# scenarios/VAE-2

Hardware: AMD Instinct MI355X
Metric: training frames/sec on 128x256 8-frame Cityscapes clips, 1/2/4/8 MI355X (higher is better)
Workload: dtype fp32; 1 GPU; VAE2 ELBO step (encz + encoder + 2 decoders fwd/bwd + Adam), HRNet-W18-small-v2, 128x256, 8 clips/GPU x 9 frames (CLIP_LENGTH=3); yaml=vae-2_amd/experiments/vae2_w18_small_v2_128x256.yaml, global_batch=8, frames_per_clip=9, parallelism=dp1, sync_bn=False, launch=hip_graph, mfma_operands=fp32

## Files before the change

### include/vae2_hip.h

```cpp
#ifndef VAE2_HIP_H
#define VAE2_HIP_H

#include <stdint.h>

#ifdef __cplusplus
extern "C" {
#endif

typedef struct vae2_act {
  int64_t n, h, w, c;
  int64_t ps;
} vae2_act;

#define VAE2_ABI_VERSION 15

int vae2_abi_version(void);
const char* vae2_last_error(void);

int vae2_kernel_log(int enable);
int64_t vae2_kernel_log_read(char* buf, int64_t len);


int64_t vae2_conv2d_fwd_stats_rows(const float* x, const vae2_act* xd, const vae2_act* yd,
                                   int k, int stride, int pad);
// ... 157 lines not shown
} vae2_bn_layer;
int vae2_bn_multi_apply(int n, const vae2_bn_layer* layers, void* stream);
int vae2_bn_multi_bwd_reduce(int n, const vae2_bn_layer* layers, void* stream);
int vae2_bn_multi_bwd_apply(int n, const vae2_bn_layer* layers, void* stream);

typedef struct vae2_bn_fin {
  const float* partials; int64_t rows; int64_t c;
  double* sums;
  const double* countp;
  double count;
  const float* gamma; const float* beta;
  float* running_mean; float* running_var; int64_t* num_batches_tracked;
  float momentum, eps;
  float* save;
  float* dgamma; float* dbeta;
} vae2_bn_fin;
int vae2_bn_multi_reduce(int n, const vae2_bn_fin* fins, int mode, void* stream);
int vae2_bn_multi_finalize(int n, const vae2_bn_fin* fins, void* stream);

int64_t vae2_conv1x1_upsum_stats_rows(const vae2_act* yd);
int vae2_conv1x1_upsum_fwd(const float* x, const vae2_act* xd, const float* wp,
                           const float* bias, int nup, const float* const* ups,
                           const vae2_act* upds, float* y, const vae2_act* yd, float* stats,
                           void* stream);

int vae2_head_out_fwd(const float* y, const vae2_act* yd, const float* save, const float* w2,
                      const float* b2, int cout2, float* out, const vae2_act* outd,
                      void* stream);
int64_t vae2_head_out_bwd_ws_size(const vae2_act* yd, int cout2);
int vae2_head_out_bwd_reduce(const float* y, const vae2_act* yd, const float* save,
                             const float* w2, int cout2, const float* dout,
                             const vae2_act* doutd, double* sums, float* dgamma, float* dbeta,
                             float* dw2, float* db2, float* ws, int64_t ws_size, void* stream);
int vae2_head_out_bwd_apply(const float* y, const vae2_act* yd, const float* save,
                            const float* gamma, const float* w2, int cout2, const float* dout,
                            const vae2_act* doutd, const double* sums, double count, float* dy,
                            const vae2_act* dyd, float* dbias, float* ws, int64_t ws_size,
                            void* stream);


int vae2_upsample_bilinear_fwd(const float* x, const vae2_act* xd, float* y,
                               const vae2_act* yd, float beta, void* stream);
int vae2_upsample_bilinear_bwd(const float* dy, const vae2_act* dyd, float* dx,
                               const vae2_act* dxd, float beta, void* stream);

int vae2_fuse_sum_relu(int n, const float* const* xs, const vae2_act* xds,
                       float* y, const vae2_act* yd, void* stream);
int vae2_fuse_sum_relu_bn(int n, const float* const* xs, const vae2_act* xds,
                          const float* const* saves, float* y, const vae2_act* yd,
                          void* stream);

int vae2_heads_set_algo(int algo);

int64_t vae2_upsample_bilinear_bwd_multi_ws_size(const vae2_act* dyd, int n,
                                                 const vae2_act* dxds);
int vae2_upsample_bilinear_bwd_multi(const float* dy, const vae2_act* dyd, int n,
                                     float* const* dxs, const vae2_act* dxds, float* ws,
                                     int64_t ws_size, void* stream);

int64_t vae2_upsample_bilinear_bwd_pow2_ws_size(const vae2_act* dyd, int n,
                                                const vae2_act* dxds);
int vae2_upsample_bilinear_bwd_pow2(const float* dy, const vae2_act* dyd, int n,
                                    float* const* dxs, const vae2_act* dxds,
                                    const float* betas, float* ws, int64_t ws_size,
                                    void* stream);

int vae2_relu_bwd(const float* dy, const vae2_act* dyd, const float* y,
                  const vae2_act* yd, float* g, const vae2_act* gd,
                  void* stream);

int vae2_relu_bwd_dual(const float* dy, const vae2_act* dyd, const float* y,
                       const vae2_act* yd, float* g, const vae2_act* gd, float* g2,
                       const vae2_act* g2d, float beta2, void* stream);

int vae2_copy_act(const float* x, const vae2_act* xd, float* y,
                  const vae2_act* yd, float beta, void* stream);

int vae2_codemap_tile_fwd(const float* v, int64_t vs, float* y,
                          const vae2_act* yd, void* stream);
int64_t vae2_spatial_ws_size(const vae2_act* xd);
int vae2_codemap_tile_bwd(const float* dy, const vae2_act* dyd, float* dv,
                          int64_t vs, int accumulate, float* ws, int64_t ws_size,
                          void* stream);

int vae2_nchw_to_nhwc(const float* x, float* y, const vae2_act* yd,
                      float beta, void* stream);
int vae2_nhwc_to_nchw(const float* x, const vae2_act* xd, float* y,
                      float beta, void* stream);

int vae2_global_avgpool_fwd(const float* x, const vae2_act* xd, float* y,
                            const vae2_act* yd, float* ws, int64_t ws_size,
                            void* stream);
int vae2_global_avgpool_bwd(const float* dy, const vae2_act* dyd, float* dx,
                            const vae2_act* dxd, float beta, void* stream);
int vae2_weighted_avgpool_fwd(const float* x, const vae2_act* xd, const float* wr,
                              const float* wc, float scale, float* y, const vae2_act* yd,
                              float* ws, int64_t ws_size, void* stream);
int vae2_weighted_avgpool_bwd(const float* dy, const vae2_act* dyd, const float* wr,
                              const float* wc, float scale, float* dx, const vae2_act* dxd,
                              float beta, void* stream);


int64_t vae2_reduce_ws_size(int64_t n);
int vae2_l1_fwd(const float* p, const vae2_act* pd, const float* t,
                const vae2_act* td, float scale, float* ws, float* out,
                void* stream);
// ... 107 lines not shown
```

### vae-2_amd/csrc/heads.hip

```cpp
#include "common.h"

namespace vae2 {


constexpr int kHeadMaxOut = 4;
constexpr int64_t kHeadMaxPpb = 2048;

template <int CO>
__device__ __forceinline__ void head_stage_dout(float* sd, const float* dout, const Act& dod,
                                                int64_t p0, int64_t p1) {
  const int n = (int)(p1 - p0) * CO;
  for (int i = threadIdx.x; i < n; i += 256) {
    const int pp = i / CO, o = i - pp * CO;
    sd[i] = dout[(p0 + pp) * dod.ps + o];
  }
}

__device__ __forceinline__ f4 hld4(const float* p) { return *reinterpret_cast<const f4*>(p); }

__device__ __forceinline__ const float* yb_at(const float* y, int64_t P, int64_t p, int c) {
  return y + (int64_t)(c >> 6) * P * 64 + p * 64 + (c & 63);
}

__device__ __forceinline__ f4 hchan4(const float* a, int c, int C) {
// ... 1072 lines not shown
int adj3_fuse_launch(const float* dy, const vae2_act* dyd, int n, float* const* dxs,
                     const vae2_act* dxds, const float* betas, hipStream_t st) {
  if (!g_adj_fused || !g_fuse_adj3 || n < 1 || n > 3 || !adj_one_pass(dyd, n, dxds)) return -1;
  for (int s = 0; s < n; ++s)
    if (!dxs[s] || dxds[s].n != dyd->n || dxds[s].c != dyd->c) return -1;
  UpAdj p{};
  p.dy = dy; p.dy_ps = (int)dyd->ps; p.H = (int)dyd->h; p.W = (int)dyd->w; p.C = (int)dyd->c;
  for (int s = 0; s < n; ++s) {
    p.dx[s] = dxs[s]; p.zh[s] = (int)dxds[s].h; p.zw[s] = (int)dxds[s].w;
    p.dx_ps[s] = (int)dxds[s].ps;
    p.beta[s] = betas ? betas[s] : 0.f;
  }
  p.nxb = (int)ceil_div(dyd->w, kUsXB);
  const int br = dyd->h < g_adj_band ? (int)dyd->h : g_adj_band;
  const int nband = (int)ceil_div(dyd->h, br);
  const dim3 grid((unsigned)(dyd->n * nband * p.nxb * ceil_div(dyd->c, 64)));
  switch (n) {
    case 1: VAE2_LAUNCH(up_adj3_kernel<1>, grid, dim3(256), 0, st, p, br, nband); break;
    case 2: VAE2_LAUNCH(up_adj3_kernel<2>, grid, dim3(256), 0, st, p, br, nband); break;
    default: VAE2_LAUNCH(up_adj3_kernel<3>, grid, dim3(256), 0, st, p, br, nband); break;
  }
  return 0;
}

static int64_t head_ppb(int64_t P, int64_t blocks = 2048) {
  int64_t ppb = ceil_div(P, blocks);
  ppb = ppb < 64 ? 64 : ppb;
  return ppb > kHeadMaxPpb ? kHeadMaxPpb : ppb;
}

static bool head_args_ok(const float* y, const vae2_act* yd, int cout2) {
  return y && act_ok(yd) && ((uintptr_t)y % 16 == 0) && (yd->c + 3) / 4 <= 256 &&
         cout2 >= 1 && cout2 <= kHeadMaxOut;
}

#define HEAD_DISPATCH(CO_, KERNEL, ...)                                   \
  switch (CO_) {                                                          \
    case 1: VAE2_LAUNCH((KERNEL<1>), __VA_ARGS__); break;          \
    case 2: VAE2_LAUNCH((KERNEL<2>), __VA_ARGS__); break;          \
    case 3: VAE2_LAUNCH((KERNEL<3>), __VA_ARGS__); break;          \
    default: VAE2_LAUNCH((KERNEL<4>), __VA_ARGS__); break;         \
  }
#define HEAD_DISPATCH_U(CO_, U_, KERNEL, ...)                                  \
  if ((U_) == 4) {                                                             \
    switch (CO_) {                                                             \
      case 1: VAE2_LAUNCH((KERNEL<1, 4>), __VA_ARGS__); break;                 \
      case 2: VAE2_LAUNCH((KERNEL<2, 4>), __VA_ARGS__); break;                 \
      case 3: VAE2_LAUNCH((KERNEL<3, 4>), __VA_ARGS__); break;                 \
      default: VAE2_LAUNCH((KERNEL<4, 4>), __VA_ARGS__); break;                \
    }                                                                          \
  } else {                                                                     \
    HEAD_DISPATCH(CO_, KERNEL, __VA_ARGS__)                                    \
  }

}

using namespace vae2;

extern "C" {

int vae2_head_out_fwd(const float* y, const vae2_act* yd, const float* save, const float* w2,
                      const float* b2, int cout2, float* out, const vae2_act* outd,
                      void* stream) {
  const char* fn = "vae2_head_out_fwd";
  VAE2_REQUIRE(head_args_ok(y, yd, cout2) && save && w2 && out && act_ok(outd), fn,
               "bad arguments (y must be 16-byte aligned NHWC with ps % 4 == 0, cout2 <= 4)");
  VAE2_REQUIRE(outd->n == yd->n && outd->h == yd->h && outd->w == yd->w && outd->c >= cout2,
               fn, "output shape mismatch");
  const int c4 = (int)((yd->c + 3) / 4);
  const size_t shm = (size_t)(2 + cout2) * c4 * 16;
  const int64_t P = act_pixels(yd);
  const unsigned grid = (unsigned)(ceil_div(P, 16) < 8192 ? ceil_div(P, 16) : 8192);
  HEAD_DISPATCH(cout2, head_out_fwd_kernel, dim3(grid), dim3(256), shm, as_stream(stream), y,
                to_act(yd), save, w2, b2, out, to_act(outd));
  return check_launch(fn);
}

int64_t vae2_head_out_bwd_ws_size(const vae2_act* yd, int cout2) {
  if (!act_ok(yd)) return 0;
  const int64_t P = act_pixels(yd);
  const int64_t blocks = ceil_div(P, head_ppb(P));
  const int64_t NC = 2 * yd->c + cout2 * yd->c + cout2;
  return blocks * NC;
}

int vae2_head_out_bwd_reduce(const float* y, const vae2_act* yd, const float* save,
                             const float* w2, int cout2, const float* dout,
                             const vae2_act* doutd, double* sums, float* dgamma, float* dbeta,
                             float* dw2, float* db2, float* ws, int64_t ws_size, void* stream) {
  const char* fn = "vae2_head_out_bwd_reduce";
  VAE2_REQUIRE(head_args_ok(y, yd, cout2) && save && w2 && dout && sums && ws &&
                   act_ok(doutd), fn, "bad arguments");
  VAE2_REQUIRE(doutd->n == yd->n && doutd->h == yd->h && doutd->w == yd->w &&
                   doutd->c >= cout2, fn, "dout shape mismatch");
  VAE2_REQUIRE(ws_size >= vae2_head_out_bwd_ws_size(yd, cout2), fn, "workspace too small");
  const int C = (int)yd->c, c4 = (C + 3) / 4, rows = 256 / c4;
  const int NC = 2 * C + cout2 * C + cout2;
  const int64_t P = act_pixels(yd), ppb = head_ppb(P);
  const unsigned blocks = (unsigned)ceil_div(P, ppb);
  const size_t shm = ((size_t)rows * NC + (size_t)ppb * cout2) * sizeof(float);
  VAE2_REQUIRE(shm <= 64 * 1024, fn, "too many channels for the LDS reduction");
  HEAD_DISPATCH_U(cout2, g_head_red_u, head_out_bwd_reduce_kernel, dim3(blocks), dim3(256), shm,
                as_stream(stream), y, to_act(yd), save, w2, dout, to_act(doutd), ppb, rows, ws);
  int rc = check_launch(fn);
  if (rc) return rc;
  VAE2_LAUNCH(head_bwd_colsum_kernel, dim3((unsigned)ceil_div(NC, 64)), dim3(1024), 0,
// ... 79 lines not shown
  dim3 grid((unsigned)(yd->n * p.nrb * p.nxb * ncb));
  hipStream_t st = as_stream(stream);
  bool one = g_upsum_one && yd->w % kUsXB == 0 && p.cin4 <= 20;
  for (int s = 0; s < nup; ++s)
    one = one && yd->h == (int64_t)p.zh[s] << (s + 1) && yd->w == (int64_t)p.zw[s] << (s + 1);
  if (one) {
#define US2_LAUNCH(N)                                                                   \
  switch (p.cin4 / 4) {                                                                 \
    case 1: VAE2_LAUNCH((upsum2_kernel<N, 1>), grid, dim3(256), 0, st, p); break;       \
    case 2: VAE2_LAUNCH((upsum2_kernel<N, 2>), grid, dim3(256), 0, st, p); break;       \
    case 3: VAE2_LAUNCH((upsum2_kernel<N, 3>), grid, dim3(256), 0, st, p); break;       \
    case 4: VAE2_LAUNCH((upsum2_kernel<N, 4>), grid, dim3(256), 0, st, p); break;       \
    default: VAE2_LAUNCH((upsum2_kernel<N, 5>), grid, dim3(256), 0, st, p); break;      \
  }
    switch (nup) {
      case 0: US2_LAUNCH(0) break;
      case 1: US2_LAUNCH(1) break;
      case 2: US2_LAUNCH(2) break;
      default: US2_LAUNCH(3) break;
    }
#undef US2_LAUNCH
    return check_launch(fn);
  }
  bool tight = g_upsum_tight != 0;
  for (int s = 0; s < nup; ++s) tight = tight && p.vcols[s] <= 4 * us_vu(s, true);
  const bool kq5 = p.cin4 <= 20;
#define US_LAUNCH(N)                                                                    \
  if (tight && kq5) VAE2_LAUNCH((upsum_kernel<N, true, 5>), grid, dim3(256), shm, st, p); \
  else if (tight) VAE2_LAUNCH((upsum_kernel<N, true, 8>), grid, dim3(256), shm, st, p); \
  else VAE2_LAUNCH((upsum_kernel<N, false, 8>), grid, dim3(256), shm, st, p);
  switch (nup) {
    case 0: US_LAUNCH(0) break;
    case 1: US_LAUNCH(1) break;
    case 2: US_LAUNCH(2) break;
    default: US_LAUNCH(3) break;
  }
#undef US_LAUNCH
  return check_launch(fn);
}

int64_t vae2_upsample_bilinear_bwd_multi_ws_size(const vae2_act* dyd, int n,
                                                 const vae2_act* dxds) {
  if (!act_ok(dyd) || n < 0 || n > 3 || (n && !dxds)) return 0;
  if (adj_one_pass(dyd, n, dxds)) return 1;
  int64_t t = 0;
  for (int s = 0; s < n; ++s) t += dyd->n * dyd->h * dxds[s].w * dyd->c;
  return t > 0 ? t : 1;
}

int vae2_heads_set_algo(int algo) {
  const int prev = (g_adj_stream ? 0 : 1) | (g_upsum_tight ? 0 : 2) | (g_adj_fused ? 0 : 4) |
                   (g_upsum_one ? 0 : 8) | (g_head_red_u == 4 ? 16 : 0) |
                   (g_head_app_u == 4 ? 32 : 0) | (g_fuse_adj3 ? 64 : 0) |
                   (g_relu_dual_q ? 0 : 128) | (g_adj_band == 32 ? 0 : g_adj_band << 8);
  g_adj_stream = (algo & 1) ? 0 : 1;
  g_upsum_tight = (algo & 2) ? 0 : 1;
  g_adj_fused = (algo & 4) ? 0 : 1;
  g_upsum_one = (algo & 8) ? 0 : 1;
  g_head_red_u = (algo & 16) ? 4 : 2;
  g_head_app_u = (algo & 32) ? 4 : 2;
  g_fuse_adj3 = (algo & 64) ? 1 : 0;
  g_relu_dual_q = (algo & 128) ? 0 : 1;
  const int band = (algo >> 8) & 0xff;
  g_adj_band = band >= 8 && band % 8 == 0 ? band : 32;
  return prev;
}

int vae2_upsample_bilinear_bwd_multi(const float* dy, const vae2_act* dyd, int n,
                                     float* const* dxs, const vae2_act* dxds, float* ws,
                                     int64_t ws_size, void* stream) {
  const char* fn = "vae2_upsample_bilinear_bwd_multi";
  VAE2_REQUIRE(dy && act_ok(dyd) && n >= 0 && n <= 3 && (n == 0 || (dxs && dxds)) && ws, fn,
               "bad arguments");
  VAE2_REQUIRE(ws_size >= vae2_upsample_bilinear_bwd_multi_ws_size(dyd, n, dxds), fn,
               "workspace too small");
  if (n == 0) return 0;
  UpAdj p{};
  p.dy = dy; p.dy_ps = (int)dyd->ps; p.H = (int)dyd->h; p.W = (int)dyd->w; p.C = (int)dyd->c;
  float* hb = ws;
  float min_sw = 1.f;
  for (int s = 0; s < n; ++s) {
    const vae2_act* d = &dxds[s];
    VAE2_REQUIRE(dxs[s] && act_ok(d) && d->n == dyd->n && d->c == dyd->c && d->h <= dyd->h &&
                     d->w <= dyd->w, fn, "dx shape mismatch");
    p.dx[s] = dxs[s]; p.zh[s] = (int)d->h; p.zw[s] = (int)d->w; p.dx_ps[s] = (int)d->ps;
    p.sh[s] = (float)d->h / (float)dyd->h;
    p.sw[s] = (float)d->w / (float)dyd->w;
    VAE2_REQUIRE(2.f / p.sh[s] + 6.f <= 64.f, fn, "upsampling ratio too large (> 24)");
    if (p.sw[s] < min_sw) min_sw = p.sw[s];
    p.hb[s] = hb;
    hb += dyd->n * dyd->h * d->w * dyd->c;
  }
  p.nxb = (int)ceil_div(dyd->w, kUsXB);
  const unsigned cb = (unsigned)ceil_div(dyd->c, 64);
  hipStream_t st = as_stream(stream);
  bool pow2 = dyd->w % kUsXB == 0;
  for (int s = 0; s < n; ++s)
    pow2 = pow2 && dyd->w == (int64_t)p.zw[s] << (s + 1) && dyd->h == (int64_t)p.zh[s] << (s + 1);
  if (adj_one_pass(dyd, n, dxds)) {
    const int br = dyd->h < g_adj_band ? (int)dyd->h : g_adj_band;
    const int nband = (int)ceil_div(dyd->h, br);
    const dim3 grid((unsigned)(dyd->n * nband * p.nxb * cb));
    switch (n) {
      case 1: VAE2_LAUNCH(up_adj3_kernel<1>, grid, dim3(256), 0, st, p, br, nband); break;
      case 2: VAE2_LAUNCH(up_adj3_kernel<2>, grid, dim3(256), 0, st, p, br, nband); break;
      default: VAE2_LAUNCH(up_adj3_kernel<3>, grid, dim3(256), 0, st, p, br, nband); break;
    }
    return check_launch(fn);
  }
  if (pow2) {
    const dim3 grid((unsigned)(dyd->n * dyd->h * p.nxb * cb));
    switch (n) {
      case 1: VAE2_LAUNCH(up_adj2_h_kernel<1>, grid, dim3(256), 0, st, p); break;
      case 2: VAE2_LAUNCH(up_adj2_h_kernel<2>, grid, dim3(256), 0, st, p); break;
      default: VAE2_LAUNCH(up_adj2_h_kernel<3>, grid, dim3(256), 0, st, p); break;
    }
    int rc = check_launch(fn);
    if (rc) return rc;
// ... 47 lines not shown
```

### vae-2_amd/vae2/_lib.py

```python
import ctypes
import os

import torch

_HERE = os.path.dirname(os.path.abspath(__file__))
LIB_PATH = os.environ.get("VAE2_LIB", os.path.join(_HERE, "libvae2_hip.so"))

c_i64 = ctypes.c_int64
c_int = ctypes.c_int
c_f32 = ctypes.c_float
c_f64 = ctypes.c_double
c_vp = ctypes.c_void_p


class Act(ctypes.Structure):

    _fields_ = [("n", c_i64), ("h", c_i64), ("w", c_i64), ("c", c_i64), ("ps", c_i64)]


P_ACT = ctypes.POINTER(Act)


class BnLayer(ctypes.Structure):
    _fields_ = [("x", c_vp), ("xd", Act), ("a", c_vp), ("ad", Act), ("o", c_vp), ("od", Act),
# ... 107 lines not shown
                                   c_f32, c_vp, P_ACT, c_f32, c_vp]),
    "vae2_bn_multi_apply": (c_int, [c_int, c_vp, c_vp]),
    "vae2_bn_multi_bwd_reduce": (c_int, [c_int, c_vp, c_vp]),
    "vae2_bn_multi_bwd_apply": (c_int, [c_int, c_vp, c_vp]),
    "vae2_bn_multi_reduce": (c_int, [c_int, c_vp, c_int, c_vp]),
    "vae2_bn_multi_finalize": (c_int, [c_int, c_vp, c_vp]),
    "vae2_lsgan_fwd": (c_int, [c_vp, P_ACT, c_f32, c_f32, c_vp, c_vp, c_vp]),
    "vae2_lsgan_bwd": (c_int, [c_vp, P_ACT, c_f32, c_vp, c_f32, c_vp, P_ACT, c_f32, c_vp]),
    "vae2_reparam_kl_fwd": (c_int, [c_vp, P_ACT, c_vp, P_ACT, c_vp, P_ACT, c_int, c_f32, c_vp,
                                    c_int, c_vp, c_vp]),
    "vae2_reparam_kl_bwd": (c_int, [c_vp, P_ACT, c_vp, P_ACT, c_vp, P_ACT, c_vp, c_f32, c_vp,
                                    P_ACT, c_vp]),
    "vae2_weighted_sum": (c_int, [c_int, ctypes.POINTER(c_vp), ctypes.POINTER(c_f32), c_vp,
                                  c_vp]),
    "vae2_nonfinite_check": (c_int, [c_vp, c_i64, c_vp, c_vp]),
    "vae2_adam_coeffs": (c_int, [c_vp, c_f32, c_f32, c_vp, c_vp]),
    "vae2_adam_step_dev": (c_int, [c_vp, c_vp, c_vp, c_vp, c_i64, c_vp, c_f32, c_f32, c_f32,
                                   c_f32, c_vp]),
    "vae2_adam_step": (c_int, [c_vp, c_vp, c_vp, c_vp, c_i64, c_f32, c_f32, c_f32, c_f32, c_f32,
                               c_i64, c_vp]),
    "vae2_sgd_coeffs": (c_int, [c_vp, c_f32, c_f32, c_int, c_vp, c_vp]),
    "vae2_sgd_step_dev": (c_int, [c_vp, c_vp, c_vp, c_i64, c_vp, c_f32, c_f32, c_int, c_vp]),
    "vae2_sgd_step": (c_int, [c_vp, c_vp, c_vp, c_i64, c_f32, c_f32, c_f32, c_f32, c_int, c_int,
                              c_vp]),
    "vae2_grad_norm_ws_size": (c_i64, [c_i64]),
    "vae2_grad_sumsq": (c_int, [c_vp, c_i64, c_vp, c_vp]),
    "vae2_clip_coeffs": (c_int, [c_vp, c_i64, c_f32, c_vp, c_vp]),
    "vae2_sgd_step_dev_clip": (c_int, [c_vp, c_vp, c_vp, c_i64, c_vp, c_vp, c_f32, c_f32, c_int,
                                       c_vp]),
    "vae2_adam_step_dev_clip": (c_int, [c_vp, c_vp, c_vp, c_vp, c_i64, c_vp, c_vp, c_f32, c_f32,
                                        c_f32, c_f32, c_vp]),
    "vae2_scale_dev": (c_int, [c_vp, c_i64, c_vp, c_vp]),
    "vae2_ema_coeffs": (c_int, [c_vp, c_f32, c_vp, c_vp]),
    "vae2_ema_update_dev": (c_int, [c_vp, c_vp, c_i64, c_vp, c_vp]),
    "vae2_ema_update": (c_int, [c_vp, c_vp, c_i64, c_f32, c_int, c_vp]),
    "vae2_scale": (c_int, [c_vp, c_vp, c_i64, c_f32, c_vp]),
    "vae2_syncbn_comm_bytes": (c_i64, [c_int, c_i64]),
    "vae2_syncbn_comm_init": (c_int, [c_int, c_int, c_i64, c_vp, ctypes.POINTER(c_vp)]),
    "vae2_syncbn_comm_connect": (c_int, [c_vp, c_vp]),
    "vae2_syncbn_allreduce": (c_int, [c_vp, c_vp, c_i64, c_vp]),
    "vae2_syncbn_comm_error": (c_int, [c_vp, ctypes.POINTER(c_i64)]),
    "vae2_syncbn_comm_set_timeout": (c_int, [c_vp, ctypes.c_double]),
    "vae2_syncbn_comm_destroy": (c_int, [c_vp]),
    "vae2_clip_normalize_u8": (c_int, [c_vp, c_i64, c_i64, c_i64, c_i64, c_vp, c_int,
                                       ctypes.POINTER(c_vp), c_vp]),
    "vae2_to_image": (c_int, [c_vp, c_vp, c_i64, c_i64, c_i64, c_i64,
                              ctypes.POINTER(c_f64), ctypes.POINTER(c_f64), c_vp]),
    "vae2_metrics_ws_size": (c_i64, [c_i64, c_i64, c_i64]),
    "vae2_absdiff_sqdiff_sum": (c_int, [c_vp, c_vp, c_i64, c_vp, c_vp, c_vp]),
    "vae2_ssim": (c_int, [c_vp, c_vp, c_i64, c_i64, c_i64, c_vp, c_int, c_f32, c_f32, c_vp,
                          c_vp, c_vp]),
    "vae2_avgpool2x2": (c_int, [c_vp, c_vp, c_i64, c_i64, c_i64, c_vp]),
    "vae2_heads_set_algo": (c_int, [c_int]),
    "vae2_conv2d_multi": (c_int, [c_int, c_vp, c_vp]),
    "vae2_weighted_avgpool_fwd": (c_int, [c_vp, P_ACT, c_vp, c_vp, c_f32, c_vp, P_ACT, c_vp,
                                          c_i64, c_vp]),
    "vae2_weighted_avgpool_bwd": (c_int, [c_vp, P_ACT, c_vp, c_vp, c_f32, c_vp, P_ACT, c_f32,
                                          c_vp]),
    "vae2_conv2d_set_grouping": (c_int, [c_int]),
}

ABI_VERSION = 15
_lib = None


def load():
    global _lib
    if _lib is not None:
        return _lib
    if not os.path.exists(LIB_PATH):
        raise RuntimeError(
            f"libvae2_hip.so not found at {LIB_PATH}: build it with "
            "`python -c 'import __graft_entry__ as g; g.build()'` "
            "(there is no fallback compute path)")
    lib = ctypes.CDLL(LIB_PATH)
    for name, (res, args) in _SIGS.items():
        fn = getattr(lib, name)
        fn.restype = res
        fn.argtypes = args
    if lib.vae2_abi_version() != ABI_VERSION:
        raise RuntimeError("libvae2_hip.so ABI version mismatch; rebuild it")
    _lib = lib
    return lib


def exported_symbols():
    return sorted(_SIGS)


class PackJob(ctypes.Structure):
    _fields_ = [("w", c_vp), ("out", c_vp), ("cout", ctypes.c_int32), ("cin", ctypes.c_int32),
                ("k", ctypes.c_int32), ("mode", ctypes.c_int32), ("ld", ctypes.c_int32),
                ("pad_", ctypes.c_int32)]


class ConvJob(ctypes.Structure):
    _fields_ = [("kind", ctypes.c_int32), ("k", ctypes.c_int32), ("stride", ctypes.c_int32),
                ("pad", ctypes.c_int32), ("x", c_vp), ("xd", Act), ("wp", c_vp), ("bias", c_vp),
                ("y", c_vp), ("yd", Act), ("beta", c_f32), ("stats", c_vp)]


class HipError(RuntimeError):
    pass


def check(rc):
# ... 15 lines not shown
```

### vae-2_amd/vae2/heads.py

```python
import ctypes

import torch

from . import _lib, prof
from ._lib import Act, call
from .ops import (_WS_HOLD, _all_reduce_sums, _bn_group, _defer_off, _empty, _grad_sink, act_of,
                  as_act, new_act, packed_weight_cols, ptr, stream_ptr, wgrad_batch)

_PER_HEAD = 6


def supported(heads, split):
    if not heads or any(h is None for h in heads) or not 1 <= len(split) <= 4:
        return False
    for h in heads:
        c0, bn, c3 = h[0], h[1], h[3]
        if c0.kernel_size != (1, 1) or c3.kernel_size != (1, 1) or c0.stride != (1, 1):
            return False
        if c3.stride != (1, 1) or c3.padding != (0, 0) or c0.padding != (0, 0):
            return False
        if c0.in_channels != sum(split) or c3.out_channels > 4 or bn.momentum is None:
            return False
        if c0.groups != 1 or c3.groups != 1:
            return False
# ... 120 lines not shown
        need = ctx.needs_input_grad[2 + nb:]
        for k in range(nh):
            w, b, gamma, beta, w2, b2 = ctx.params[_PER_HEAD * k:_PER_HEAD * (k + 1)]
            nw, nbias, ng, nbt, nw2, nb2 = need[_PER_HEAD * k:_PER_HEAD * (k + 1)]
            y, save = yv[k], saves[k]
            yp, ya = ptr(y), Act(*ys[0].shape[:3], C, C)
            dk = dout[..., ncls * k:ncls * (k + 1)]
            dkp, dka = act_of(dk)
            wsz = lib.vae2_head_out_bwd_ws_size(ctypes.byref(ya), ncls)
            ws = _empty((wsz,), y)
            lsums = _empty((2 * C,), y, torch.float64)
            gsink, gret = _grad_sink(gamma, ng)
            btsink, btret = _grad_sink(beta, nbt)
            w2sink, w2ret = _grad_sink(w2, nw2)
            b2sink, b2ret = _grad_sink(b2, nb2)
            P0 = ys[0].shape[0] * ys[0].shape[1] * ys[0].shape[2]
            Hh, Ww = ys[0].shape[1], ys[0].shape[2]
            if prof.active():
                prof.note(2.0 * P0 * C * ncls, 4.0 * (P0 * C + P0 * ncls),
                          prof.conv_label("head out wgrad", C, ncls, 1, 1, Hh, Ww))
            call("vae2_head_out_bwd_reduce", yp, ctypes.byref(ya), ptr(save), ptr(w2), ncls, dkp,
                 ctypes.byref(dka), ptr(lsums), ptr(gsink), ptr(btsink), ptr(w2sink),
                 ptr(b2sink), ptr(ws), wsz, s)
            gsums, _ = _all_reduce_sums(lsums, ctx.count, ctx.group)
            dy = new_act((*ys[0].shape[:3], C), y)
            dyp, dya = act_of(dy)
            bsink, bret = _grad_sink(b, nbias)
            if prof.active():
                prof.note(2.0 * P0 * C * ncls, 4.0 * (2 * P0 * C + P0 * ncls),
                          prof.conv_label("head out dgrad", C, ncls, 1, 1, Hh, Ww))
            call("vae2_head_out_bwd_apply", yp, ctypes.byref(ya), ptr(save), ptr(gamma), ptr(w2),
                 ncls, dkp, ctypes.byref(dka), ptr(gsums), ctx.count, dyp, ctypes.byref(dya),
                 ptr(bsink), ptr(ws), wsz, s)
            wsink, wret = _grad_sink(w, nw)
            gs = [(dy, dyp, dya)]
            for xj in ys[1:]:
                g = new_act((xj.shape[0], xj.shape[1], xj.shape[2], C), xj)
                gs.append((g, *act_of(g)))
            if nb > 1:
                gptrs = (ctypes.c_void_p * 3)(*[gp for _, gp, _ in gs[1:]])
                gacts = (Act * 3)(*[ga for _, _, ga in gs[1:]])
                usz = lib.vae2_upsample_bilinear_bwd_multi_ws_size(ctypes.byref(dya), nb - 1, gacts)
                uws = _empty((usz,), y)
                if prof.active():
                    prof.note(0.0, 4.0 * (dy.numel() + sum(g.numel() for g, _, _ in gs[1:])))
                call("vae2_upsample_bilinear_bwd_multi", dyp, ctypes.byref(dya), nb - 1, gptrs,
                     gacts, ptr(uws), usz, s)
            c0 = 0
            with wgrad_batch():
                for j in range(nb):
                    xj = ys[j]
                    g, gp, ga = gs[j]
                    xjp, xja = act_of(xj)
                    if wsink is not None:
                        wsz2 = lib.vae2_conv2d_bwd_weight_ws_size(ctypes.byref(xja),
                                                                  ctypes.byref(ga), 1)
                        ws2 = _empty((max(wsz2, 1),), xj)
                        if prof.active():
                            pj = xja.n * xja.h * xja.w
                            prof.note(2.0 * pj * xja.c * C, 4.0 * (pj * xja.c + pj * C + C * xja.c),
                                      prof.conv_label("head wgrad", xja.c, C, 1, 1, xja.h, xja.w))
                        with _defer_off(wret is not None):
                            call("vae2_conv2d_bwd_weight_ld", xjp, ctypes.byref(xja), gp,
                                 ctypes.byref(ga), ctypes.c_void_p(wsink.data_ptr() + 4 * c0),
                                 C, None, 1, 1, 0, 1, ptr(ws2), wsz2, s)
                        if wret is None:
                            _WS_HOLD.append((torch.cuda.current_stream().cuda_stream, ws2))
                    if ctx.needs_input_grad[2 + j]:
                        first = dxs[j] is None
                        if first:
                            dxs[j] = new_act(tuple(xj.shape), xj)
                        dxp, dxa = act_of(dxs[j])
                        if prof.active():
                            pj = dxa.n * dxa.h * dxa.w
                            prof.note(2.0 * pj * dxa.c * C, 4.0 * (pj * dxa.c + pj * C + C * dxa.c),
                                      prof.conv_label("head dgrad", dxa.c, C, 1, 1, dxa.h, dxa.w))
                        call("vae2_conv2d_bwd_data", gp, ctypes.byref(ga),
                             ptr(packed_weight_cols(w, split, j, 1)), dxp, ctypes.byref(dxa), 1,
                             1, 0, 0.0 if first else 1.0, s)
                    c0 += split[j]
            pgrads += [wret, bret, gret, btret, w2ret, b2ret]
        return (None, None, *dxs, *pgrads)


def run(heads, ys):
    params = []
    for h in heads:
        params += [h[0].weight, h[0].bias, h[1].weight, h[1].bias, h[3].weight, h[3].bias]
    return _Heads.apply(tuple(heads), len(ys), *ys, *params)
```

Before: 927.8 frames/s.

## Fuse head branch dgrad and wgrad into one warp-specialized kernel

Adds a fused backward kernel for the 1x1 head conv branches with small input channel counts (up to 18). It loads each tile of the output gradient once into LDS. Four waves compute dx with MFMA while four other waves accumulate per-block weight-gradient partials, which a second kernel reduces in double precision. This replaces the separate dgrad and wgrad launches, which each re-read the large gradient tensor, and uses double-buffered register prefetch. The cost is a workspace slab per block, an extra reduce launch, and heavy LDS use that limits occupancy.

```diff
diff --git a/include/vae2_hip.h b/include/vae2_hip.h
--- a/include/vae2_hip.h
+++ b/include/vae2_hip.h
@@ -233,6 +233,12 @@
 
 int vae2_heads_set_algo(int algo);
 
+int64_t vae2_head_branch_bwd_ws_size(const vae2_act* gd, const vae2_act* xd);
+int vae2_head_branch_bwd(const float* g, const vae2_act* gd, const float* x,
+                         const vae2_act* xd, const float* w, int64_t ld, float* dx,
+                         const vae2_act* dxd, float beta, float* dw, int accumulate, float* ws,
+                         int64_t ws_size, void* stream);
+
 int64_t vae2_upsample_bilinear_bwd_multi_ws_size(const vae2_act* dyd, int n,
                                                  const vae2_act* dxds);
 int vae2_upsample_bilinear_bwd_multi(const float* dy, const vae2_act* dyd, int n,
diff --git a/vae-2_amd/csrc/heads.hip b/vae-2_amd/csrc/heads.hip
--- a/vae-2_amd/csrc/heads.hip
+++ b/vae-2_amd/csrc/heads.hip
@@ -1148,6 +1148,291 @@
   } else {                                                                     \
     HEAD_DISPATCH(CO_, KERNEL, __VA_ARGS__)                                    \
   }
+
+constexpr int kHbPx = 64, kHbLd = 276, kHbXs = 20, kHbRows = 272, kHbR = 2;
+constexpr int kHbSlab = (kHbRows + 48) * kHbXs;
+constexpr int kHbMaxGrid = 256;
+static int g_head_branch = 1;
+static int g_head_branch_grid = 0;
+
+__device__ __forceinline__ uint32_t hb_off(uint32_t a, uint32_t b) {
+  return (a + b) | ((a | b) & kOOB);
+}
+
+struct HeadBranch {
+  const float* g;
+  const float* x;
+  const float* w;
+  float* dx;
+  float* part;
+  uint32_t g_bytes, x_bytes, w_bytes, dx_bytes;
+  int g_ps, x_ps, w_ld, dx_ps;
+  int C, cin, P, ntiles;
+  float beta;
+};
+
+__global__ __launch_bounds__(512) void head_branch_bwd_kernel(HeadBranch p) {
+  __shared__ __attribute__((aligned(16))) float gs[kHbPx * kHbLd];
+  __shared__ __attribute__((aligned(16))) float xs[kHbPx * kHbXs];
+  __shared__ __attribute__((aligned(16))) float wrs[kHbR * kHbRows];
+  const int tid = threadIdx.x, lane = tid & 63;
+  const int wave = __builtin_amdgcn_readfirstlane(tid >> 6);
+  const int g = lane >> 4, r = lane & 15;
+  const __amdgpu_buffer_rsrc_t gr = make_rsrc(p.g, p.g_bytes);
+  const __amdgpu_buffer_rsrc_t xr = make_rsrc(p.x, p.x_bytes);
+  const int c4 = (p.C + 3) >> 2;
+  f4 gn0[9], gn1[9];
+  float xn0[3], xn1[3];
+  const int lq = tid & 15, lp = tid >> 4;
+  uint32_t qo[5], xo[3];
+#pragma unroll
+  for (int m = 0; m < 4; ++m) qo[m] = lq + 16 * m < c4 ? 16u * (lq + 16 * m) : kOOB;
+  qo[4] = (tid < 256 && 64 + (tid & 3) < c4) ? 16u * (64 + (tid & 3)) : kOOB;
+#pragma unroll
+  for (int i = 0; i < 3; ++i) {
+    const int e = tid + 512 * i, pp = e / kHbXs, k = e - pp * kHbXs;
+    xo[i] = (e < kHbPx * kHbXs && k < p.cin) ? 4u * k : kOOB;
+  }
+  auto issue = [&](int tile, f4 (&gn)[9], float (&xn)[3]) {
+    const int p0 = tile * kHbPx;
+#pragma unroll
+    for (int n = 0; n < 2; ++n) {
+      const int px = p0 + lp + 32 * n;
+      const uint32_t ro = px < p.P ? (uint32_t)px * (uint32_t)p.g_ps * 4u : kOOB;
+#pragma unroll
+      for (int m = 0; m < 4; ++m) gn[4 * n + m] = load4(gr, hb_off(ro, qo[m]));
+    }
+    {
+      const int px = p0 + (tid >> 2);
+      gn[8] = load4(gr, hb_off(px < p.P ? (uint32_t)px * (uint32_t)p.g_ps * 4u : kOOB, qo[4]));
+    }
+#pragma unroll
+    for (int i = 0; i < 3; ++i) {
+      const int px = p0 + (tid + 512 * i) / kHbXs;
+      xn[i] = load1(xr, hb_off(px < p.P ? (uint32_t)px * (uint32_t)p.x_ps * 4u : kOOB, xo[i]));
+    }
+  };
+  auto put = [&](int px, int cq, f4 v) {
+#pragma unroll
+    for (int i = 0; i < 4; ++i) v[i] = 4 * cq + i < p.C ? v[i] : 0.f;
+    *reinterpret_cast<f4*>(gs + px * kHbLd + 4 * cq) = v;
+  };
+  auto commit = [&](const f4 (&gn)[9], const float (&xn)[3]) {
+#pragma unroll
+    for (int n = 0; n < 2; ++n)
+#pragma unroll
+      for (int m = 0; m < 4; ++m) put(lp + 32 * n, lq + 16 * m, gn[4 * n + m]);
+    if (tid < 256) put(tid >> 2, 64 + (tid & 3), gn[8]);
+#pragma unroll
+    for (int i = 0; i < 3; ++i)
+      if (tid + 512 * i < kHbPx * kHbXs) xs[tid + 512 * i] = xn[i];
+  };
+  if (wave < 4) {
+    const __amdgpu_buffer_rsrc_t wr = make_rsrc(p.w, p.w_bytes);
+    const __amdgpu_buffer_rsrc_t dxr = make_rsrc(p.dx, p.dx ? p.dx_bytes : 0u);
+    float wf[17][4];
+#pragma unroll
+    for (int u = 0; u < 17; ++u)
+#pragma unroll
+      for (int i = 0; i < 4; ++i) {
+        const int c = 16 * u + 4 * g + i;
+        wf[u][i] = load1(wr, (p.dx && c < p.C && r < p.cin) ? (uint32_t)(c * p.w_ld + r) * 4u
+                                                             : kOOB);
+      }
+    for (int e = tid; e < kHbR * kHbRows; e += 256) {
+      const int kr = e / kHbRows, c = e - kr * kHbRows;
+      wrs[e] = load1(wr, (c < p.C && 16 + kr < p.cin) ? (uint32_t)(c * p.w_ld + 16 + kr) * 4u
+                                                      : kOOB);
+    }
+    __builtin_amdgcn_s_waitcnt(0x0F70);
+    issue(blockIdx.x, gn0, xn0);
+    __builtin_amdgcn_sched_barrier(0);
+    issue(blockIdx.x + gridDim.x, gn1, xn1);
+    __builtin_amdgcn_sched_barrier(0);
+    const int nq = p.cin - 4 * g < 0 ? 0 : (p.cin - 4 * g > 4 ? 4 : p.cin - 4 * g);
+    const float* grow = gs + (16 * wave + r) * kHbLd + 4 * g;
+    const float* wrow = wrs + 4 * g;
+    auto step = [&](int tile, f4 (&gn)[9], float (&xn)[3]) {
+      __syncthreads();
+      commit(gn, xn);
+      __syncthreads();
+      const int pg = tile * kHbPx + 16 * wave + r;
+      const bool pok = p.dx && pg < p.P;
+      const uint32_t dxo = ((uint32_t)pg * (uint32_t)p.dx_ps + 4u * g) * 4u;
+      const uint32_t dro = ((uint32_t)pg * (uint32_t)p.dx_ps + 16u) * 4u;
+      const bool old = pok && p.beta != 0.f;
+      const f4 o4 = load4(dxr, old && nq > 0 ? dxo : kOOB);
+      float o1[kHbR];
+#pragma unroll
+      for (int kr = 0; kr < kHbR; ++kr)
+        o1[kr] = load1(dxr, old && g == 0 && 16 + kr < p.cin ? dro + 4u * kr : kOOB);
+      __builtin_amdgcn_sched_barrier(0);
+      issue(tile + 2 * gridDim.x, gn, xn);
+      if (!p.dx) return;
+      f4 a0 = f4{0.f, 0.f, 0.f, 0.f}, a1 = a0;
+      float ar[kHbR];
+#pragma unroll
+      for (int kr = 0; kr < kHbR; ++kr) ar[kr] = 0.f;
+#pragma unroll
+      for (int u = 0; u < 17; ++u) {
+        const f4 v = *reinterpret_cast<const f4*>(grow + 16 * u);
+#pragma unroll
+        for (int i = 0; i < 4; ++i) {
+          if (u & 1) a1 = __builtin_amdgcn_mfma_f32_16x16x4f32(wf[u][i], v[i], a1, 0, 0, 0);
+          else a0 = __builtin_amdgcn_mfma_f32_16x16x4f32(wf[u][i], v[i], a0, 0, 0, 0);
+        }
+#pragma unroll
+        for (int kr = 0; kr < kHbR; ++kr) {
+          const f4 wq = *reinterpret_cast<const f4*>(wrow + kr * kHbRows + 16 * u);
+#pragma unroll
+          for (int i = 0; i < 4; ++i) ar[kr] = __builtin_fmaf(v[i], wq[i], ar[kr]);
+        }
+      }
+#pragma unroll
+      for (int kr = 0; kr < kHbR; ++kr) {
+        ar[kr] += __shfl_xor(ar[kr], 16, 64);
+        ar[kr] += __shfl_xor(ar[kr], 32, 64);
+      }
+      f4 d = a0 + a1;
+#pragma unroll
+      for (int i = 0; i < 4; ++i) d[i] = __builtin_fmaf(p.beta, o4[i], d[i]);
+      store_quad(dxr, pok ? dxo : kOOB, d, nq);
+#pragma unroll
+      for (int kr = 0; kr < kHbR; ++kr)
+        store1(dxr, pok && g == 0 && 16 + kr < p.cin ? dro + 4u * kr : kOOB,
+               __builtin_fmaf(p.beta, o1[kr], ar[kr]));
+    };
+    for (int tile = blockIdx.x; tile < p.ntiles; tile += 2 * gridDim.x) {
+      step(tile, gn0, xn0);
+      step(tile + gridDim.x, gn1, xn1);
+    }
+  } else {
+    const int w4 = wave - 4;
+    f4 aw[5];
+    float awr[5][kHbR];
+#pragma unroll
+    for (int jj = 0; jj < 5; ++jj) {
+      aw[jj] = f4{0.f, 0.f, 0.f, 0.f};
+#pragma unroll
+      for (int kr = 0; kr < kHbR; ++kr) awr[jj][kr] = 0.f;
+    }
+    const float* gcol = gs + 4 * g * kHbLd + 16 * w4 + r;
+    const float* xrow = xs + 4 * g * kHbXs;
+    const float* gcol16 = gs + (16 * w4 + 4 * g) * kHbLd + 256 + r;
+    const float* xrow16 = xs + (16 * w4 + 4 * g) * kHbXs;
+    issue(blockIdx.x, gn0, xn0);
+    __builtin_amdgcn_sched_barrier(0);
+    issue(blockIdx.x + gridDim.x, gn1, xn1);
+    __builtin_amdgcn_sched_barrier(0);
+    auto step = [&](int tile, f4 (&gn)[9], float (&xn)[3]) {
+      __syncthreads();
+      commit(gn, xn);
+      __syncthreads();
+      issue(tile + 2 * gridDim.x, gn, xn);
+      if (!p.part) return;
+#pragma unroll 4
+      for (int s = 0; s < 16; ++s) {
+        const int px = 16 * (s >> 2) + (s & 3);
+        const float b = xrow[px * kHbXs + r];
+        float xv[kHbR];
+#pragma unroll
+        for (int kr = 0; kr < kHbR; ++kr) xv[kr] = xrow[px * kHbXs + 16 + kr];
+#pragma unroll
+        for (int jj = 0; jj < 4; ++jj) {
+          const float a = gcol[px * kHbLd + 64 * jj];
+          aw[jj] = __builtin_amdgcn_mfma_f32_16x16x4f32(a, b, aw[jj], 0, 0, 0);
+#pragma unroll
+          for (int kr = 0; kr < kHbR; ++kr) awr[jj][kr] = __builtin_fmaf(a, xv[kr], awr[jj][kr]);
+        }
+      }
+#pragma unroll
+      for (int t = 0; t < 4; ++t) {
+        const float b = xrow16[t * kHbXs + r];
+        const float a = gcol16[t * kHbLd];
+        aw[4] = __builtin_amdgcn_mfma_f32_16x16x4f32(a, b, aw[4], 0, 0, 0);
+#pragma unroll
+        for (int kr = 0; kr < kHbR; ++kr)
+          awr[4][kr] = __builtin_fmaf(a, xrow16[t * kHbXs + 16 + kr], awr[4][kr]);
+      }
+    };
+    for (int tile = blockIdx.x; tile < p.ntiles; tile += 2 * gridDim.x) {
+      step(tile, gn0, xn0);
+      step(tile + gridDim.x, gn1, xn1);
+    }
+    if (p.part) {
+      float* slab = p.part + (int64_t)blockIdx.x * kHbSlab;
+#pragma unroll
+      for (int jj = 0; jj < 5; ++jj) {
+        const int j = w4 + 4 * jj;
+#pragma unroll
+        for (int e = 0; e < 4; ++e) slab[(16 * j + 4 * g + e) * kHbXs + r] = aw[jj][e];
+#pragma unroll
+        for (int kr = 0; kr < kHbR; ++kr) {
+          float v = awr[jj][kr];
+          v += __shfl_xor(v, 16, 64);
+          v += __shfl_xor(v, 32, 64);
+          if (g == 0) slab[(16 * j + r) * kHbXs + 16 + kr] = v;
+        }
+      }
+    }
+  }
+}
+
+__global__ __launch_bounds__(1024) void head_branch_dw_reduce_kernel(
+    const float* __restrict__ part, int nslab, int C, int cin, float* __restrict__ dw, int ld,
+    int accumulate) {
+  __shared__ double red[16][64];
+  const int lane = threadIdx.x & 63, wave = threadIdx.x >> 6;
+  const int col = blockIdx.x * 64 + lane, NC = C * cin;
+  const int c = col / cin, k = col - c * cin;
+  double s0 = 0.0, s1 = 0.0, s2 = 0.0, s3 = 0.0;
+  if (col < NC) {
+    const float* src = part + c * kHbXs + k;
+    const int nq = c >= 256 ? 4 : 1;
+    for (int q = 0; q < nq; ++q, src += 16 * kHbXs) {
+      int i = wave;
+      for (; i + 48 < nslab; i += 64) {
+        s0 += (double)src[(int64_t)i * kHbSlab];
+        s1 += (double)src[(int64_t)(i + 16) * kHbSlab];
+        s2 += (double)src[(int64_t)(i + 32) * kHbSlab];
+        s3 += (double)src[(int64_t)(i + 48) * kHbSlab];
+      }
+      for (; i < nslab; i += 16) s0 += (double)src[(int64_t)i * kHbSlab];
+    }
+  }
+  red[wave][lane] = (s0 + s1) + (s2 + s3);
+  __syncthreads();
+  if (wave != 0 || col >= NC) return;
+  double s = 0.0;
+#pragma unroll
+  for (int w = 0; w < 16; ++w) s += red[w][lane];
+  float* o = dw + (int64_t)c * ld + k;
+  *o = accumulate ? *o + (float)s : (float)s;
+}
+
+extern int g_bf16;
+
+static bool head_branch_ok(const vae2_act* gd, const vae2_act* xd) {
+  if (!g_head_branch || g_bf16 || !act_ok(gd) || !act_ok(xd)) return false;
+  if (gd->n != xd->n || gd->h != xd->h || gd->w != xd->w) return false;
+  const int64_t P = act_pixels(gd);
+  if (xd->c > 16 + kHbR || gd->c > kHbRows || (gd->ps % 4 != 0 && P > 1)) return false;
+  return P * gd->ps * 4 < (1ll << 31) && P * xd->ps * 4 < (1ll << 31);
+}
+
+static int head_branch_grid(int64_t ntiles) {
+  static int per_cu = 0;
+  if (!per_cu) {
+    int n = 0;
+    if (hipOccupancyMaxActiveBlocksPerMultiprocessor(
+            &n, reinterpret_cast<const void*>(head_branch_bwd_kernel), 512, 0) != hipSuccess)
+      n = 1;
+    per_cu = n < 1 ? 1 : n;
+  }
+  int64_t grid = g_head_branch_grid > 0 ? g_head_branch_grid : 256 * per_cu;
+  if (grid > kHbMaxGrid) grid = kHbMaxGrid;
+  return (int)(grid < ntiles ? grid : ntiles);
+}
 
 }
 
@@ -1333,7 +1618,8 @@
   const int prev = (g_adj_stream ? 0 : 1) | (g_upsum_tight ? 0 : 2) | (g_adj_fused ? 0 : 4) |
                    (g_upsum_one ? 0 : 8) | (g_head_red_u == 4 ? 16 : 0) |
                    (g_head_app_u == 4 ? 32 : 0) | (g_fuse_adj3 ? 64 : 0) |
-                   (g_relu_dual_q ? 0 : 128) | (g_adj_band == 32 ? 0 : g_adj_band << 8);
+                   (g_relu_dual_q ? 0 : 128) | (g_adj_band == 32 ? 0 : g_adj_band << 8) |
+                   (g_head_branch ? 0 : 1 << 16) | (g_head_branch_grid << 17);
   g_adj_stream = (algo & 1) ? 0 : 1;
   g_upsum_tight = (algo & 2) ? 0 : 1;
   g_adj_fused = (algo & 4) ? 0 : 1;
@@ -1344,7 +1630,52 @@
   g_relu_dual_q = (algo & 128) ? 0 : 1;
   const int band = (algo >> 8) & 0xff;
   g_adj_band = band >= 8 && band % 8 == 0 ? band : 32;
+  g_head_branch = (algo & (1 << 16)) ? 0 : 1;
+  const int hb_grid = (algo >> 17) & 0x3ff;
+  g_head_branch_grid = hb_grid <= kHbMaxGrid ? hb_grid : kHbMaxGrid;
   return prev;
+}
+
+int64_t vae2_head_branch_bwd_ws_size(const vae2_act* gd, const vae2_act* xd) {
+  return head_branch_ok(gd, xd) ? (int64_t)kHbMaxGrid * kHbSlab : 0;
+}
+
+int vae2_head_branch_bwd(const float* g, const vae2_act* gd, const float* x,
+                         const vae2_act* xd, const float* w, int64_t ld, float* dx,
+                         const vae2_act* dxd, float beta, float* dw, int accumulate, float* ws,
+                         int64_t ws_size, void* stream) {
+  const char* fn = "vae2_head_branch_bwd";
+  VAE2_REQUIRE(head_branch_ok(gd, xd), fn,
+               "unsupported case (vae2_head_branch_bwd_ws_size returns 0 for it)");
+  VAE2_REQUIRE(g && x && w && (dx || dw) && (uintptr_t)g % 16 == 0 && ld >= xd->c &&
+                   ld < (1 << 20), fn, "bad arguments (g must be 16-byte aligned)");
+  VAE2_REQUIRE(!dx || (act_ok(dxd) && dxd->n == xd->n && dxd->h == xd->h && dxd->w == xd->w &&
+                       dxd->c == xd->c && (dxd->ps % 4 == 0 || act_pixels(dxd) == 1) &&
+                       (uintptr_t)dx % 16 == 0 &&
+                       act_pixels(dxd) * dxd->ps * 4 < (1ll << 31)), fn,
+               "dx shape mismatch (x's shape, 16-byte aligned pixels)");
+  VAE2_REQUIRE(!dw || (ws && ws_size >= (int64_t)kHbMaxGrid * kHbSlab), fn,
+               "workspace too small");
+  HeadBranch p{};
+  const int64_t P = act_pixels(gd);
+  p.g = g; p.x = x; p.w = w; p.dx = dx; p.part = dw ? ws : nullptr;
+  p.g_bytes = (uint32_t)(((P - 1) * gd->ps + (gd->c + 3) / 4 * 4) * 4);
+  p.x_bytes = (uint32_t)(((P - 1) * xd->ps + xd->c) * 4);
+  p.w_bytes = (uint32_t)(((gd->c - 1) * ld + xd->c) * 4);
+  p.dx_bytes = dx ? (uint32_t)(P * dxd->ps * 4) : 0u;
+  p.g_ps = (int)gd->ps; p.x_ps = (int)xd->ps; p.w_ld = (int)ld;
+  p.dx_ps = dx ? (int)dxd->ps : 0;
+  p.C = (int)gd->c; p.cin = (int)xd->c; p.P = (int)P;
+  p.ntiles = (int)ceil_div(P, kHbPx);
+  p.beta = beta;
+  const int grid = head_branch_grid(p.ntiles);
+  hipStream_t st = as_stream(stream);
+  VAE2_LAUNCH(head_branch_bwd_kernel, dim3((unsigned)grid), dim3(512), 0, st, p);
+  int rc = check_launch(fn);
+  if (rc || !dw) return rc;
+  VAE2_LAUNCH(head_branch_dw_reduce_kernel, dim3((unsigned)ceil_div(p.C * p.cin, 64)),
+              dim3(1024), 0, st, (const float*)ws, grid, p.C, p.cin, dw, (int)ld, accumulate);
+  return check_launch(fn);
 }
 
 int vae2_upsample_bilinear_bwd_multi(const float* dy, const vae2_act* dyd, int n,
diff --git a/vae-2_amd/vae2/_lib.py b/vae-2_amd/vae2/_lib.py
--- a/vae-2_amd/vae2/_lib.py
+++ b/vae-2_amd/vae2/_lib.py
@@ -183,6 +183,9 @@
                           c_vp, c_vp]),
     "vae2_avgpool2x2": (c_int, [c_vp, c_vp, c_i64, c_i64, c_i64, c_vp]),
     "vae2_heads_set_algo": (c_int, [c_int]),
+    "vae2_head_branch_bwd_ws_size": (c_i64, [P_ACT, P_ACT]),
+    "vae2_head_branch_bwd": (c_int, [c_vp, P_ACT, c_vp, P_ACT, c_vp, c_i64, c_vp, P_ACT, c_f32,
+                                     c_vp, c_int, c_vp, c_i64, c_vp]),
     "vae2_conv2d_multi": (c_int, [c_int, c_vp, c_vp]),
     "vae2_weighted_avgpool_fwd": (c_int, [c_vp, P_ACT, c_vp, c_vp, c_f32, c_vp, P_ACT, c_vp,
                                           c_i64, c_vp]),
diff --git a/vae-2_amd/vae2/heads.py b/vae-2_amd/vae2/heads.py
--- a/vae-2_amd/vae2/heads.py
+++ b/vae-2_amd/vae2/heads.py
@@ -196,6 +196,33 @@
                     xj = ys[j]
                     g, gp, ga = gs[j]
                     xjp, xja = act_of(xj)
+                    need_dx = ctx.needs_input_grad[2 + j]
+                    fsz = lib.vae2_head_branch_bwd_ws_size(ctypes.byref(ga), ctypes.byref(xja))
+                    if fsz > 0 and (wsink is not None or need_dx):
+                        first = dxs[j] is None
+                        if need_dx and first:
+                            dxs[j] = new_act(tuple(xj.shape), xj)
+                        dxp, dxa = act_of(dxs[j]) if need_dx else (None, xja)
+                        fws = _empty((fsz,), xj) if wsink is not None else None
+                        if prof.active():
+                            pj, cj = xja.n * xja.h * xja.w, xja.c
+                            nprod = (wsink is not None) + bool(need_dx)
+                            nby = pj * C + pj * cj + C * cj
+                            if need_dx:
+                                nby += pj * cj * (1 if first else 2)
+                            if wsink is not None:
+                                nby += 2 * C * cj + 2 * fsz
+                            prof.note(2.0 * pj * cj * C * nprod, 4.0 * nby,
+                                      prof.conv_label("head dgrad+wgrad" if nprod == 2 else
+                                                      "head dgrad" if need_dx else "head wgrad",
+                                                      cj, C, 1, 1, xja.h, xja.w))
+                        call("vae2_head_branch_bwd", gp, ctypes.byref(ga), xjp, ctypes.byref(xja),
+                             ctypes.c_void_p(w.data_ptr() + 4 * c0), C, dxp, ctypes.byref(dxa),
+                             0.0 if first else 1.0,
+                             ctypes.c_void_p(wsink.data_ptr() + 4 * c0) if wsink is not None
+                             else None, 1, ptr(fws), fsz, s)
+                        c0 += split[j]
+                        continue
                     if wsink is not None:
                         wsz2 = lib.vae2_conv2d_bwd_weight_ws_size(ctypes.byref(xja),
                                                                   ctypes.byref(ga), 1)
@@ -210,7 +237,7 @@
                                  C, None, 1, 1, 0, 1, ptr(ws2), wsz2, s)
                         if wret is None:
                             _WS_HOLD.append((torch.cuda.current_stream().cuda_stream, ws2))
-                    if ctx.needs_input_grad[2 + j]:
+                    if need_dx:
                         first = dxs[j] is None
                         if first:
                             dxs[j] = new_act(tuple(xj.shape), xj)
```

After: 935.5 frames/s, median of 6. About the same (+0.8%).
